# Adamtaranto/mimeo

Measured on AMD Instinct MI355X. Metric: Gbp-aligned/sec (mimeo self, 1 Gbp genome, --minIdt 80 --minLen 100 --minCov 3), higher is better.
Workload: dtype int32

## Files before the change

mimeo_amd/csrc/k6_gapped.hip:

```cpp
#include <algorithm>
#include <cstdio>
#include <cstdlib>
#include <cstring>
#include <vector>

#include "device_util.h"

namespace mimeo {

constexpr int32_t NEG = -(1 << 30);
constexpr int32_t NEGH = -(1 << 29);

struct Cell {
    int32_t s;
    uint32_t nm, nx;
};
struct HalfResult {
    int32_t score;
    uint32_t i, j, nm, nx, overflow;
    uint32_t maxcols, rows;
    uint32_t base_lo, base_hi;
};
struct DpJob {
    uint32_t group, at, aq;
// ... 522 lines not shown
        const int32_t cs = max(hs, is);
        const uint32_t cc = ins ? acc.c : hc;
        const bool take = hs > acc.s;
        acc.c = take ? hc : acc.c;
        acc.s = max(acc.s, hs) - E;
        bool alive = cs >= thr;
        if (EDGE) alive = alive && ((exmask >> s) & 1u);
        S.C[s] = alive ? cs : NEG; S.Cc[s] = cc;
        S.D[s] = alive ? S.D[s] : NEG;
        rowmax = max(rowmax, S.C[s]);
    }
    return rowmax;
}

__device__ HalfResult wave_half_extend_lean(const StrandView &T, const StrandView &Q, uint32_t at, uint32_t aq, int dir,
                                            int32_t O, int32_t E, int32_t Y) {
    const uint32_t lane = threadIdx.x & 63u;
    const uint32_t lenA = dir > 0 ? T.len - at : at, lenB = dir > 0 ? Q.len - aq : aq;
    HalfResult best{0, 0, 0, 0, 0, 0, 0, 0};
    {
        const uint32_t n = min(lenA, lenB);
        const int32_t st = dir > 0 ? (int32_t)at : (int32_t)(at - n), sq = dir > 0 ? (int32_t)aq : (int32_t)(aq - n);
        bool ok = true;
        uint64_t ncg = 0;
        for (uint32_t k0 = 0; k0 < n; k0 += 64u * 32u) {
            uint32_t k = k0 + lane * 32u;
            if (k < n) {
                const Win32 tw = win32(T, st + (int32_t)k), qw = win32(Q, sq + (int32_t)k);
                uint32_t bad = (tw.lo ^ qw.lo) | (tw.hi ^ qw.hi) | tw.nm | qw.nm;
                uint32_t rem = n - k, mask = rem < 32 ? (1u << rem) - 1u : 0xFFFFFFFFu;
                if (bad & mask) ok = false;
                ncg += __popc((tw.lo ^ tw.hi) & mask);
            }
            if (__ballot(!ok)) break;
        }
        if (!__ballot(!ok)) {
            for (int o = 32; o > 0; o >>= 1) ncg += __shfl_xor(ncg, o);
            uint64_t sc = 100ull * ncg + 91ull * ((uint64_t)n - ncg);
            best.score = (int32_t)(uint32_t)sc; best.maxcols = (uint32_t)(sc >> 32); best.i = n; best.j = n; best.nm = n; best.nx = 0;
            return best;
        }
    }
    uint32_t tab[4];
#pragma unroll
    for (uint32_t a = 0; a < 4; a++) {
        uint32_t w = 0;
#pragma unroll
        for (uint32_t b = 0; b < 4; b++) {
            const uint32_t alo = a & 1u, ahi = a >> 1, dl = alo ^ (b & 1u), dh = ahi ^ (b >> 1);
            w |= (uint32_t)(sub_score(dl, dh, alo ^ ahi, 0u) + 128) << (8u * b);
        }
        tab[a] = w;
    }
    LeanState S;
    uint32_t wb = 0, jb = lane * L_WS;
    {
        uint32_t qlo, qhi, qn;
        load_qbits<L_WS>(Q, aq, dir, jb, lenB, qlo, qhi, qn);
        lean_selectors(S, qlo, qhi, qn);
    }
    bool over = false;
#pragma unroll
    for (int s = 0; s < L_WS; s++) {
        const uint32_t j = jb + s;
        const int32_t v = j ? -O - (int32_t)j * E : 0;
        const bool alive = j <= lenB && (j == 0 || v >= -Y);
        S.C[s] = alive ? v : NEG; S.Cc[s] = 0;
        S.D[s] = NEG; S.Dc[s] = 0;
        if (alive && j >= (uint32_t)(L_WINDOW - L_WS)) over = true;
    }
    if (__ballot(over)) { best.overflow = 1; return best; }
    const int32_t lane_base = (int32_t)(lane * L_WS) * E;
    const int32_t kneg128 = __builtin_amdgcn_readfirstlane(-128);
    uint32_t exmask = (1u << L_WS) - 1u;
    bool edge = wb + (uint32_t)L_WINDOW - 1u > lenB;
    if (edge) {
        exmask = 0;
#pragma unroll
        for (int s = 0; s < L_WS; s++) exmask |= (jb + s <= lenB ? 1u : 0u) << s;
    }
    RowBases rbase{0, 0, 0}, rnext = load_row_bases(T, at, dir, 1u);
    for (uint32_t i = 1; i <= lenA; i++) {
        if (i >= 0xFFFFu) { best.overflow = 1; break; }
        const int32_t thr = best.score - Y;
        const uint32_t rbit = (i - 1u) & 31u;
        if (rbit == 0) { rbase = rnext; rnext = load_row_bases(T, at, dir, i + 32u); }
        const uint32_t rlo = (uint32_t)__builtin_amdgcn_readfirstlane((int)rbase.lo), rhi = (uint32_t)__builtin_amdgcn_readfirstlane((int)rbase.hi),
                       rnm = (uint32_t)__builtin_amdgcn_readfirstlane((int)rbase.nm);
        const uint32_t a = ((rlo >> rbit) & 1u) | (((rhi >> rbit) & 1u) << 1);
        uint32_t srow = a & 2u ? (a & 1u ? tab[3] : tab[2]) : (a & 1u ? tab[1] : tab[0]);
        if ((rnm >> rbit) & 1u) srow = 0x1C1C1C1Cu;
        const int32_t rowmax = edge ? lean_row<true>(S, srow, O, E, thr, exmask, lane_base, kneg128)
                                    : lean_row<false>(S, srow, O, E, thr, exmask, lane_base, kneg128);
        const uint64_t ball = __ballot(rowmax > NEGH);
        if (!ball) break;
        const uint32_t rf = (uint32_t)__builtin_ctzll(ball), rl = 63u - (uint32_t)__builtin_clzll(ball);
        if (rl == 63u) { best.overflow = 1; break; }
        best.maxcols = max(best.maxcols, (rl + 1u) * L_WS);
        best.rows = i;
        const int32_t wmax = wave_max_i32(rowmax);
        if (wmax > best.score) {
            const uint32_t L = (uint32_t)__builtin_ctzll(__ballot(rowmax == wmax));
            uint32_t slot = 0, cnt = 0;
#pragma unroll
            for (int s = L_WS - 1; s >= 0; s--) {
                const int32_t v = __builtin_amdgcn_readlane(S.C[s], (int)L);
                if (v == wmax) { slot = (uint32_t)s; cnt = (uint32_t)__builtin_amdgcn_readlane((int)S.Cc[s], (int)L); }
            }
            best.score = wmax; best.i = i; best.j = wb + L * L_WS + slot; best.nm = cnt & 0xFFFFu; best.nx = (cnt >> 16) - (cnt & 0xFFFFu);
        }
        if (rf) {
            wb += rf * L_WS;
            jb = wb + lane * L_WS;
            const int src = (int)((lane + rf) & 63u);
            const bool fresh = lane + rf >= 64u;
#pragma unroll
            for (int s = 0; s < L_WS; s++) {
                const int32_t cs = __shfl(S.C[s], src), ds = __shfl(S.D[s], src);
                S.Cc[s] = __shfl(S.Cc[s], src); S.Dc[s] = __shfl(S.Dc[s], src);
                S.sel[s] = __shfl(S.sel[s], src);
                S.C[s] = fresh ? NEG : cs;
                S.D[s] = fresh ? NEG : ds;
            }
            if (fresh) {
                uint32_t qlo, qhi, qn;
                load_qbits<L_WS>(Q, aq, dir, jb, lenB, qlo, qhi, qn);
                lean_selectors(S, qlo, qhi, qn);
            }
            edge = wb + (uint32_t)L_WINDOW - 1u > lenB;
            if (edge) {
                exmask = 0;
#pragma unroll
                for (int s = 0; s < L_WS; s++) exmask |= (jb + s <= lenB ? 1u : 0u) << s;
            }
        }
    }
    return best;
}

__global__ __launch_bounds__(64) void k6_dp1(const Group *__restrict__ groups, const DpJob *__restrict__ jobs,
                                             HalfResult *__restrict__ res, int32_t O, int32_t E, int32_t Y) {
    const DpJob job = jobs[blockIdx.x];
    const Group &G = groups[job.group];
    HalfResult r = wave_half_extend_lean(G.T, G.Q, job.at, job.aq, job.dir, O, E, Y);
    if (threadIdx.x == 0) res[job.slot] = r;
}

__global__ __launch_bounds__(C4_THREADS) void k6_dp4(const Group *__restrict__ groups, const DpJob *__restrict__ jobs,
                                                     HalfResult *__restrict__ res, int32_t O, int32_t E, int32_t Y) {
    __shared__ C4Shared sh;
    const DpJob job = jobs[blockIdx.x];
    const Group &G = groups[job.group];
    HalfResult r = block_half_extend(sh, G.T, G.Q, job.at, job.aq, job.dir, O, E, Y);
    if (threadIdx.x == 0) res[job.slot] = r;
}

constexpr uint32_t ANCHOR_W = 31, ANCHOR_CHUNK = 4096;
constexpr int ANCHOR_THREADS = 1024;

__device__ void wave_anchor_chunk(const StrandView &T, const StrandView &Q, const mimeo_hsp &h, uint32_t chunk,
                                  unsigned long long *packed) {
    const uint32_t lane = threadIdx.x & 63u, nw = h.length - ANCHOR_W + 1;
    const int32_t d = (int32_t)h.tstart - (int32_t)h.qstart;
    const uint32_t w0 = chunk * ANCHOR_CHUNK + lane * (ANCHOR_CHUNK / 64u), w1 = min(nw, w0 + ANCHOR_CHUNK / 64u);
    int32_t bs = INT32_MIN;
    uint32_t bw = 0xFFFFFFFFu;
    if (w0 < w1) {
        int32_t sum = 0;
        bool m;
        for (uint32_t k = 0; k < ANCHOR_W; k++) {
            int32_t pt = (int32_t)(h.tstart + w0 + k);
            sum += pair_score(T, Q, pt, pt - d, &m);
        }
        bs = sum; bw = w0;
        for (uint32_t w = w0 + 1; w < w1; w++) {
            int32_t add = (int32_t)(h.tstart + w + ANCHOR_W - 1), sub = (int32_t)(h.tstart + w - 1);
            sum += pair_score(T, Q, add, add - d, &m) - pair_score(T, Q, sub, sub - d, &m);
            if (sum > bs) { bs = sum; bw = w; }
        }
    }
    for (int o = 32; o > 0; o >>= 1) {
        int32_t ob = __shfl_xor(bs, o);
        uint32_t ow = __shfl_xor(bw, o);
        if (ob > bs || (ob == bs && ow < bw)) { bs = ob; bw = ow; }
    }
    if (lane == 0 && bw != 0xFFFFFFFFu)
        atomicMax(packed, ((unsigned long long)(uint32_t)(bs + 8192) << 32) | (unsigned long long)(0xFFFFFFFFu - bw));
}

constexpr uint32_t ANCHOR_SPLIT = 16;
__global__ __launch_bounds__(ANCHOR_THREADS) void k6_anchor_points(const Group *__restrict__ groups,
                                                                   const mimeo_hsp *__restrict__ hs,
                                                                   const uint32_t *__restrict__ order,
                                                                   unsigned long long *__restrict__ packed) {
    const Group &G = groups[blockIdx.x];
    const uint64_t b0 = G.hsp_begin;
    const uint32_t nw = gridDim.y * (ANCHOR_THREADS / 64), me = blockIdx.y * (ANCHOR_THREADS / 64) + (threadIdx.x >> 6);
    uint32_t item = 0;
    for (uint32_t r = 0; r < G.nchain; r++) {
        const mimeo_hsp h = hs[b0 + order[b0 + r]];
        if (h.length <= ANCHOR_W) continue;
        const uint32_t nch = (h.length - ANCHOR_W + 1 + ANCHOR_CHUNK - 1) / ANCHOR_CHUNK;
        const uint32_t first = (me + nw - item % nw) % nw;
        for (uint32_t c = first; c < nch; c += nw) wave_anchor_chunk(G.T, G.Q, h, c, &packed[b0 + r]);
        item += nch;
    }
}
__global__ __launch_bounds__(256) void k6_anchor_final(const Group *__restrict__ groups, const mimeo_hsp *__restrict__ hs,
                                                       const uint32_t *__restrict__ order,
                                                       const unsigned long long *__restrict__ packed,
                                                       uint2 *__restrict__ anchors) {
    const Group &G = groups[blockIdx.x];
    const uint64_t b0 = G.hsp_begin;
    for (uint32_t r = threadIdx.x; r < G.nchain; r += blockDim.x) {
        const mimeo_hsp h = hs[b0 + order[b0 + r]];
        uint32_t off = h.length / 2;
        if (h.length > ANCHOR_W) off = (0xFFFFFFFFu - (uint32_t)packed[b0 + r]) + ANCHOR_W / 2;
        anchors[b0 + r] = make_uint2(h.tstart + off, h.qstart + off);
    }
}

__device__ __forceinline__ bool in_boxes(const mimeo_alignment *aln, uint32_t n, uint2 a) {
    bool inside = false;
    for (uint32_t e = threadIdx.x & 63u; e < n; e += 64u) {
        const mimeo_alignment &o = aln[e];
        if (a.x >= o.tstart && a.x < o.tend && a.y >= o.qstart && a.y < o.qend) inside = true;
    }
    return __ballot(inside) != 0;
}

struct PathBlock {
    uint32_t t, q, len;
};
constexpr uint32_t PATH_UNTRACED = 0xFFFFFFFFu;
struct PathView {
    const uint2 *pidx;
    const PathBlock *blk;
    uint32_t *accrank;
};
__device__ __forceinline__ bool on_half_path(const PathBlock *blk, uint32_t n, uint2 a) {
    uint32_t lo = 0, hi = n;
    while (lo < hi) {
        const uint32_t mid = (lo + hi) >> 1;
        if (blk[mid].t <= a.x) lo = mid + 1; else hi = mid;
    }
    if (!lo) return false;
    const PathBlock b = blk[lo - 1];
    return a.x - b.t < b.len && a.y >= b.q && a.y - b.q == a.x - b.t;
}
__device__ __forceinline__ bool on_path(const PathView &P, const uint2 *anchors, uint64_t b0, uint32_t rank, uint2 a) {
    const uint2 an = anchors[b0 + rank];
    const uint2 ix = P.pidx[2u * (b0 + rank) + (a.x >= an.x ? 1u : 0u)];
    if (ix.x == PATH_UNTRACED) return false;
    return on_half_path(P.blk + ix.x, ix.y, a);
}
template <bool PATH>
__device__ __forceinline__ bool skip_test(const mimeo_alignment *aln, uint32_t n, uint2 a, const PathView &P,
                                          const uint2 *anchors, uint64_t b0) {
    if (!PATH) return in_boxes(aln + b0, n, a);
    bool on = false;
    for (uint32_t e = threadIdx.x & 63u; e < n; e += 64u) {
        const mimeo_alignment &o = aln[b0 + e];
        if (a.x >= o.tstart && a.x < o.tend && a.y >= o.qstart && a.y < o.qend && on_path(P, anchors, b0, P.accrank[b0 + e], a))
            on = true;
    }
    return __ballot(on) != 0;
}

enum : uint8_t { A_NEW = 0, A_DONE = 1, A_SKIPPED = 2, A_ACCEPTED = 3 };
constexpr uint32_t PICK_SCAN = 512;
constexpr uint32_t NEAR_DIAG = 256, NEAR_POS = 8192, MAX_DEFER = 2;

__device__ __forceinline__ bool anchors_near(uint2 a, uint2 b) {
    int32_t da = (int32_t)a.x - (int32_t)a.y, db = (int32_t)b.x - (int32_t)b.y;
    uint32_t dd = (uint32_t)abs(da - db), dp = a.x > b.x ? a.x - b.x : b.x - a.x;
    return dd <= NEAR_DIAG && dp <= NEAR_POS;
}

template <bool PATH>
__global__ __launch_bounds__(64) void k6_pick(Group *__restrict__ groups, const uint2 *__restrict__ anchors,
                                              const mimeo_alignment *__restrict__ aln, uint32_t bmax,
                                              uint8_t *__restrict__ astate, uint8_t *__restrict__ adefer,
                                              DpJob *__restrict__ jobs, unsigned int *__restrict__ njobs, PathView P) {
    __shared__ uint32_t sb[MAX_BATCH];
    Group &G = groups[blockIdx.x];
    const uint64_t b0 = G.hsp_begin;
    const uint32_t first = G.next, lane = threadIdx.x;
    uint32_t nb = 0;
    for (uint32_t r = first; r < G.nchain && nb < bmax && r - first < PICK_SCAN; r++) {
        if (astate[b0 + r] != A_NEW) continue;
        const uint2 a = anchors[b0 + r];
        if (skip_test<PATH>(aln, G.nacc, a, P, anchors, b0)) {
            if (lane == 0) astate[b0 + r] = A_SKIPPED;
            continue;
        }
        bool susp = false;
        for (uint32_t r2 = first + lane; r2 < r; r2 += 64)
            if (astate[b0 + r2] == A_DONE && anchors_near(a, anchors[b0 + r2])) susp = true;
        if (lane < nb && anchors_near(a, anchors[b0 + sb[lane]])) susp = true;
        if (__ballot(susp) && adefer[b0 + r] < MAX_DEFER) {
            if (lane == 0) adefer[b0 + r]++;
            continue;
        }
        if (lane == 0) sb[nb] = r;
        nb++;
        __syncthreads();
// ... 481 lines not shown
            m.tid = G.tid; m.qid = G.qid; m.qstrand = G.minus; m.reserved = 0;
            m.tstart = h.tstart; m.tend = h.tstart + h.length; m.qstart = h.qstart; m.qend = h.qstart + h.length;
            m.score = h.score; m.id_n = nmatch; m.id_d = h.length;
            aln[b0 + r] = m;
        }
    }
    if (threadIdx.x == 0) G.nacc = G.nchain;
}

__global__ void k6_finish(Group *__restrict__ groups, uint32_t ngroups, mimeo_alignment *__restrict__ aln,
                          int32_t thresh) {
    uint32_t g = blockIdx.x * blockDim.x + threadIdx.x;
    if (g >= ngroups) return;
    Group &G = groups[g];
    const uint64_t b0 = G.hsp_begin;
    uint32_t k = 0;
    for (uint32_t e = 0; e < G.nacc; e++) {
        mimeo_alignment a = aln[b0 + e];
        if (a.score < thresh) continue;
        if (G.minus) { uint32_t s = G.Q.len - a.qend, t2 = G.Q.len - a.qstart; a.qstart = s; a.qend = t2; }
        aln[b0 + k++] = a;
    }
    G.naln = k;
}

__global__ __launch_bounds__(1024) void k6_dense_offsets(Group *__restrict__ groups, uint32_t ngroups) {
    __shared__ uint32_t part[1024];
    __shared__ uint32_t carry;
    if (threadIdx.x == 0) carry = 0;
    __syncthreads();
    for (uint32_t g0 = 0; g0 < ngroups; g0 += 1024) {
        const uint32_t g = g0 + threadIdx.x, n = g < ngroups ? groups[g].naln : 0u;
        part[threadIdx.x] = n;
        __syncthreads();
        for (uint32_t o = 1; o < 1024; o <<= 1) {
            const uint32_t v = threadIdx.x >= o ? part[threadIdx.x - o] : 0u;
            __syncthreads();
            part[threadIdx.x] += v;
            __syncthreads();
        }
        if (g < ngroups) groups[g].job0 = carry + part[threadIdx.x] - n;
        __syncthreads();
        if (threadIdx.x == 1023) carry += part[1023];
        __syncthreads();
    }
}
__global__ __launch_bounds__(64) void k6_dense_copy(const Group *__restrict__ groups, const mimeo_alignment *__restrict__ aln,
                                                    mimeo_alignment *__restrict__ dense) {
    const Group &G = groups[blockIdx.x];
    for (uint32_t k = threadIdx.x; k < G.naln; k += 64) dense[G.job0 + k] = aln[G.hsp_begin + k];
}
void dense_alignments_device(Group *d_groups, uint32_t ngroups, const mimeo_alignment *d_aln, mimeo_alignment *d_dense) {
    hipLaunchKernelGGL(k6_dense_offsets, dim3(1), dim3(1024), 0, stream(), d_groups, ngroups);
    hipLaunchKernelGGL(k6_dense_copy, dim3(ngroups), dim3(64), 0, stream(), (const Group *)d_groups, d_aln, d_dense);
}

static DeviceBuf g_anchors, g_packed, g_jobs, g_res, g_cnt, g_astate, g_ovf_list, g_any;
static DeviceBuf g_pidx, g_accrank, g_arena, g_pool, g_tjobs, g_tres, g_tctr;

static int trace_pool_budget(uint64_t *budget) {
    size_t free_b = 0, total_b = 0;
    HIP_TRY(hipMemGetInfo(&free_b, &total_b));
    *budget = std::min<uint64_t>(((uint64_t)free_b + g_pool.cap) / 4, 16ull << 30);
    if (getenv("MIMEO_K6_TRACE_POOL_MB")) *budget = (uint64_t)atol(getenv("MIMEO_K6_TRACE_POOL_MB")) << 20;
    return 0;
}

static int arena_reserve(uint64_t blocks, uint64_t used) {
    const size_t bytes = (size_t)blocks * sizeof(PathBlock);
    if (bytes <= g_arena.cap) return 0;
    DeviceBuf nb;
    int rc = nb.reserve(std::max(bytes, 2 * g_arena.cap));
    if (rc) return rc;
    if (used) HIP_TRY(hipMemcpyAsync(nb.p, g_arena.p, (size_t)used * sizeof(PathBlock), hipMemcpyDeviceToDevice, stream()));
    HIP_TRY(hipStreamSynchronize(stream()));
    g_arena.release();
    g_arena = nb;
    return 0;
}

static int trace_round(Group *d_groups, uint32_t h0, const mimeo_params *p, uint64_t budget, uint64_t *arena_used, float *ms,
                       uint32_t *slices, uint64_t *largest) {
    hipStream_t st = stream();
    int rc;
    if ((rc = g_tres.reserve((size_t)h0 * sizeof(HalfResult)))) return rc;
    hipLaunchKernelGGL(k6_trace_gather, dim3((h0 + 255) / 256), dim3(256), 0, st, (const DpJob *)g_jobs.p, h0, (const HalfResult *)g_res.p,
                       (HalfResult *)g_tres.p);
    std::vector<HalfResult> hr(h0);
    HIP_TRY(hipMemcpyAsync(hr.data(), g_tres.p, (size_t)h0 * sizeof(HalfResult), hipMemcpyDeviceToHost, st));
    HIP_TRY(hipStreamSynchronize(st));
    const int32_t O = p->gap_open, E = p->gap_extend, Y = p->ydrop;
    const uint32_t ext = (uint32_t)((Y + 200) / E) + 2u, hi0 = Y >= O + E ? (uint32_t)((Y - O) / E) : 0u;
    std::vector<TraceJob> tj(h0);
    std::vector<uint32_t> cut{0};
    uint64_t fill = 0, need_max = 0, blocks = 0;
    for (uint32_t k = 0; k < h0; k++) {
        const HalfResult &r = hr[k];
        TraceJob J{0, 0, 0, TR_NONE, 0};
        if (!r.overflow && r.i) {
            if (r.rows == 0) { J.mode = TR_DIAG; blocks += 1; }
            else {
                J.W = std::max(r.maxcols, hi0 + 1u) + ext + 2u;
                J.R = 1u;
                while (J.R < J.W + 2u) J.R <<= 1;
                J.cap = std::min(r.i, r.j) + 1u;
                const uint64_t need = trace_layout(r.i, J.W, J.R, J.cap).total;
                *largest = std::max(*largest, need);
                if (need > budget) J.mode = TR_UNTRACED;
                else {
                    J.mode = TR_DP;
                    blocks += J.cap;
                    if (fill + need > budget) { cut.push_back(k); fill = 0; }
                    J.off = fill;
                    fill += need;
                    need_max = std::max(need_max, fill);
                }
            }
        }
        tj[k] = J;
    }
    cut.push_back(h0);
    if ((rc = g_tjobs.reserve((size_t)h0 * sizeof(TraceJob)))) return rc;
    HIP_TRY(hipMemcpyAsync(g_tjobs.p, tj.data(), (size_t)h0 * sizeof(TraceJob), hipMemcpyHostToDevice, st));
    if (need_max && (rc = g_pool.reserve(need_max))) return rc;
    if ((rc = arena_reserve(*arena_used + blocks + 1, *arena_used))) return rc;
    static hipEvent_t e0 = nullptr, e1 = nullptr;
    if (!e0) { HIP_TRY(hipEventCreate(&e0)); HIP_TRY(hipEventCreate(&e1)); }
    HIP_TRY(hipEventRecord(e0, st));
    for (size_t c = 0; c + 1 < cut.size(); c++)
        if (cut[c + 1] > cut[c] && ++*slices)
            hipLaunchKernelGGL(k6_trace, dim3(cut[c + 1] - cut[c]), dim3(TR_THREADS), 0, st, (const Group *)d_groups,
                               (const DpJob *)g_jobs.p, (const TraceJob *)g_tjobs.p, cut[c], (const HalfResult *)g_res.p,
                               (uint8_t *)g_pool.p, (PathBlock *)g_arena.p, (unsigned long long)(g_arena.cap / sizeof(PathBlock)),
                               (uint2 *)g_pidx.p, (unsigned int *)g_tctr.p, O, E, Y);
    HIP_TRY(hipEventRecord(e1, st));
    unsigned int c3[3] = {0, 0, 0};
    HIP_TRY(hipMemcpyAsync(c3, g_tctr.p, 12, hipMemcpyDeviceToHost, st));
    HIP_TRY(hipStreamSynchronize(st));
    float t = 0;
    HIP_TRY(hipEventElapsedTime(&t, e0, e1));
    *ms += t;
    if (c3[1]) {
        char msg[200];
        snprintf(msg, sizeof msg, "internal: K6 traceback of half slot %u %s", c3[2],
                 c3[1] == TRERR_DP ? "disagrees with its DP result (score or end cell)"
                 : c3[1] == TRERR_WALK ? "disagrees with its DP result (matches / mismatches along the path)" : "outgrew the block arena");
        set_error(msg);
        return MIMEO_ERR_ARG;
    }
    *arena_used = c3[0];
    return 0;
}

int gapped_device(Group *d_groups, uint32_t ngroups, const mimeo_hsp *d_sorted, const uint32_t *d_order,
                  uint64_t nhsps, const mimeo_params *p, mimeo_alignment *d_aln) {
    if (!ngroups || !nhsps) return 0;
    hipStream_t st = stream();
    int rc;
    if (!p->gapped) {
        hipLaunchKernelGGL(k6_ungapped, dim3(ngroups), dim3(256), 0, st, d_groups, d_sorted, d_order, d_aln);
    } else {
        uint32_t bmax = 8192u / ngroups;
        if (getenv("MIMEO_K6_BMAX")) bmax = (uint32_t)atoi(getenv("MIMEO_K6_BMAX"));
        const char *kmode = getenv("MIMEO_K6_KERNEL");
        const bool k6_stats = getenv("MIMEO_K6_STATS") != nullptr;
        const int32_t cap = getenv("MIMEO_K6_SCORE_CAP") ? std::max(100000, atoi(getenv("MIMEO_K6_SCORE_CAP"))) : 2000000000;
        bmax = bmax < 1 ? 1 : (bmax > MAX_BATCH ? MAX_BATCH : bmax);
        if ((rc = g_anchors.reserve(nhsps * sizeof(uint2)))) return rc;
        if ((rc = g_packed.reserve(nhsps * 8))) return rc;
        HIP_TRY(hipMemsetAsync(g_packed.p, 0, nhsps * 8, st));
        if ((rc = g_jobs.reserve((size_t)ngroups * bmax * 2 * sizeof(DpJob)))) return rc;
        if ((rc = g_res.reserve((size_t)nhsps * 2 * sizeof(HalfResult)))) return rc;
        if ((rc = g_astate.reserve((size_t)nhsps * 2))) return rc;
        HIP_TRY(hipMemsetAsync(g_astate.p, 0, (size_t)nhsps * 2, st));
        if ((rc = g_cnt.reserve(16))) return rc;
        if ((rc = g_ovf_list.reserve((size_t)ngroups * bmax * 2 * sizeof(unsigned int)))) return rc;
        const uint32_t asplit = ngroups > 4096 ? 1u : ANCHOR_SPLIT;
        hipLaunchKernelGGL(k6_anchor_points, dim3(ngroups, asplit), dim3(ANCHOR_THREADS), 0, st, (const Group *)d_groups,
                           d_sorted, d_order, (unsigned long long *)g_packed.p);
        hipLaunchKernelGGL(k6_anchor_final, dim3(ngroups), dim3(256), 0, st, (const Group *)d_groups, d_sorted, d_order,
                           (const unsigned long long *)g_packed.p, (uint2 *)g_anchors.p);
        const bool path = p->anchor_rule == MIMEO_ANCHOR_PATH;
        uint64_t pool_budget = 0, arena_used = 0;
        float ms_trace = 0;
        uint32_t trace_slices = 0, rounds = 0;
        uint64_t largest = 0;
        PathView pv{nullptr, nullptr, nullptr};
        if (path) {
            if ((rc = g_pidx.reserve((size_t)nhsps * 2 * sizeof(uint2)))) return rc;
            if ((rc = g_accrank.reserve((size_t)nhsps * 4))) return rc;
            if ((rc = g_tctr.reserve(16))) return rc;
            if ((rc = arena_reserve(1024, 0))) return rc;
            HIP_TRY(hipMemsetAsync(g_tctr.p, 0, 16, st));
            if ((rc = trace_pool_budget(&pool_budget))) return rc;
            pv = PathView{(const uint2 *)g_pidx.p, nullptr, (uint32_t *)g_accrank.p};
        }
        for (;;) {
            HIP_TRY(hipMemsetAsync(g_cnt.p, 0, 16, st));
            unsigned int *njobs = (unsigned int *)g_cnt.p, *remaining = njobs + 1, *novf = njobs + 2;
            pv.blk = (const PathBlock *)g_arena.p;
            if (path)
                hipLaunchKernelGGL(k6_pick<true>, dim3(ngroups), dim3(64), 0, st, d_groups, (const uint2 *)g_anchors.p,
                                   (const mimeo_alignment *)d_aln, bmax, (uint8_t *)g_astate.p, (uint8_t *)g_astate.p + nhsps,
                                   (DpJob *)g_jobs.p, njobs, pv);
            else
                hipLaunchKernelGGL(k6_pick<false>, dim3(ngroups), dim3(64), 0, st, d_groups, (const uint2 *)g_anchors.p,
                                   (const mimeo_alignment *)d_aln, bmax, (uint8_t *)g_astate.p, (uint8_t *)g_astate.p + nhsps,
                                   (DpJob *)g_jobs.p, njobs, pv);
            unsigned int h[2] = {0, 0};
            HIP_TRY(hipMemcpyAsync(h, g_cnt.p, 4, hipMemcpyDeviceToHost, st));
            HIP_TRY(hipStreamSynchronize(st));
            if (h[0]) {
                const bool lean_ok = p->gap_extend <= (1 << 16) && p->gap_open <= (1 << 24) && p->ydrop <= (1 << 28);
                if (lean_ok && !kmode) {
                    hipLaunchKernelGGL(k6_dp1, dim3(h[0]), dim3(64), 0, st, (const Group *)d_groups, (const DpJob *)g_jobs.p,
                                       (HalfResult *)g_res.p, p->gap_open, p->gap_extend, p->ydrop);
                } else {
                    const bool use4 = !kmode || !strcmp(kmode, "dp4");
                    if (use4)
                        hipLaunchKernelGGL(k6_dp4, dim3(h[0]), dim3(C4_THREADS), 0, st, (const Group *)d_groups,
                                           (const DpJob *)g_jobs.p, (HalfResult *)g_res.p, p->gap_open, p->gap_extend, p->ydrop);
                    hipLaunchKernelGGL(k6_dp, dim3(h[0]), dim3(64), 0, st, (const Group *)d_groups, (const DpJob *)g_jobs.p,
                                       (HalfResult *)g_res.p, p->gap_open, p->gap_extend, p->ydrop, use4 ? 1 : 0, cap);
                }
                hipLaunchKernelGGL(k6_dp_wide, dim3(h[0]), dim3(64), 0, st, (const Group *)d_groups,
                                   (const DpJob *)g_jobs.p, (HalfResult *)g_res.p, p->gap_open, p->gap_extend, p->ydrop, novf,
                                   (unsigned int *)g_ovf_list.p, cap);
                unsigned int nov = 0;
                HIP_TRY(hipMemcpyAsync(&nov, novf, 4, hipMemcpyDeviceToHost, st));
                HIP_TRY(hipStreamSynchronize(st));
                if (nov) {
                    const unsigned int slots = std::min<unsigned int>(nov, 32u);
                    if ((rc = g_any.reserve((size_t)slots * ANY_SLOT_WORDS * 4))) return rc;
                    for (unsigned int f = 0; f < nov; f += slots)
                        hipLaunchKernelGGL(k6_dp_any, dim3(std::min(slots, nov - f)), dim3(ANY_THREADS), 0, st, (const Group *)d_groups,
                                           (const DpJob *)g_jobs.p, (const unsigned int *)g_ovf_list.p, f, (HalfResult *)g_res.p,
                                           (uint32_t *)g_any.p, p->gap_open, p->gap_extend, p->ydrop, cap);
                }
            }
            if (k6_stats && h[0]) {
                std::vector<DpJob> hj(h[0]);
                std::vector<HalfResult> hall((size_t)nhsps * 2), hr(h[0]);
                HIP_TRY(hipStreamSynchronize(st));
                HIP_TRY(hipMemcpy(hj.data(), g_jobs.p, (size_t)h[0] * sizeof(DpJob), hipMemcpyDeviceToHost));
                HIP_TRY(hipMemcpy(hall.data(), g_res.p, hall.size() * sizeof(HalfResult), hipMemcpyDeviceToHost));
                for (size_t k = 0; k < hr.size(); k++) hr[k] = hall[hj[k].slot];
                unsigned long long hist[9] = {0}, rows = 0, maxr = 0, shortcut = 0;
                for (auto &r : hr) {
                    if (!r.rows) { shortcut++; continue; }
                    hist[std::min<uint32_t>(8, r.maxcols / 128)]++; rows += r.rows; maxr = std::max<unsigned long long>(maxr, r.rows);
                }
                unsigned long long rebased = 0;
                for (auto &r : hr) if (r.base_lo | r.base_hi) rebased++;
                fprintf(stderr, "[k6] jobs %u shortcut %llu (rebased in k6_dp_any: %llu) rows total %llu max %llu band<128..>=1024:", h[0], shortcut, rebased, rows, maxr);
                for (int b = 0; b < 9; b++) fprintf(stderr, " %llu", hist[b]);
                fprintf(stderr, "\n");
                {
                    unsigned long long fine[34] = {0};
                    for (auto &r : hr) if (r.rows) fine[std::min<uint32_t>(33, r.maxcols / 32)]++;
                    fprintf(stderr, "[k6] widest band, buckets of 32 columns from 448:");
                    for (int b = 14; b < 34; b++) fprintf(stderr, " %llu", fine[b]);
                    fprintf(stderr, "\n");
                }
                int shown = 0;
                for (auto &r : hr)
                    if (!r.rows && shown < 8) { fprintf(stderr, "  [k6] zero-row job: score %d i %u j %u nm %u nx %u ovf %u\n", r.score, r.i, r.j, r.nm, r.nx, r.overflow); shown++; }
            }
            if (path && h[0]) {
                rounds++;
                if ((rc = trace_round(d_groups, h[0], p, pool_budget, &arena_used, &ms_trace, &trace_slices, &largest))) return rc;
                pv.blk = (const PathBlock *)g_arena.p;
            }
            if (path)
                hipLaunchKernelGGL(k6_resolve<true>, dim3(ngroups), dim3(64), 0, st, d_groups, (const uint2 *)g_anchors.p,
                                   (const HalfResult *)g_res.p, d_aln, (uint8_t *)g_astate.p, remaining, pv);
            else
                hipLaunchKernelGGL(k6_resolve<false>, dim3(ngroups), dim3(64), 0, st, d_groups, (const uint2 *)g_anchors.p,
                                   (const HalfResult *)g_res.p, d_aln, (uint8_t *)g_astate.p, remaining, pv);
            HIP_TRY(hipMemcpyAsync(h, g_cnt.p, 8, hipMemcpyDeviceToHost, st));
            HIP_TRY(hipStreamSynchronize(st));
            if (!h[1]) break;
        }
        if (path && k6_stats)
            fprintf(stderr, "[k6] path rule: traceback %.3f ms, rounds %u slices %u, %llu path blocks, pool %.1f MB, largest half %.3f MB\n", ms_trace,
                    rounds, trace_slices, (unsigned long long)arena_used, g_pool.cap / 1048576.0, largest / 1048576.0);
    }
    hipLaunchKernelGGL(k6_finish, dim3((ngroups + 63) / 64), dim3(64), 0, st, d_groups, ngroups, d_aln, p->hspthresh);
    HIP_TRY(hipGetLastError());
    return 0;
}

}
```

Before: 0.04243.

## Add four-wave banded DP kernel for rounds with few gapped-extension jobs

Adds k6_dp1w, a 256-thread (four-wave) version of the lean half-extension DP. Each wave owns a 320-column block of a sliding 1280-column window, and the waves exchange boundaries and row maxima through shared memory. It is selected when a round has no more jobs than the device's compute-unit count, so the GPU stays busy in tail rounds where the single-wave kernel leaves most CUs idle. The cost is two block barriers per DP row and more overflow fallbacks when the band outgrows the window.

```diff
diff --git a/mimeo_amd/csrc/k6_gapped.hip b/mimeo_amd/csrc/k6_gapped.hip
--- a/mimeo_amd/csrc/k6_gapped.hip
+++ b/mimeo_amd/csrc/k6_gapped.hip
@@ -698,6 +698,244 @@
     const DpJob job = jobs[blockIdx.x];
     const Group &G = groups[job.group];
     HalfResult r = block_half_extend(sh, G.T, G.Q, job.at, job.aq, job.dir, O, E, Y);
+    if (threadIdx.x == 0) res[job.slot] = r;
+}
+
+constexpr int T_WS = 5, T_BLOCK = 64 * T_WS, T_WINDOW = 4 * T_BLOCK, T_THREADS = 256;
+struct ThinState {
+    int32_t C[T_WS], D[T_WS];
+    uint32_t Cc[T_WS], Dc[T_WS], sel[T_WS];
+};
+struct alignas(16) ThinRecord {
+    uint32_t live;
+    int32_t s;
+    uint32_t j, c;
+};
+struct ThinShared {
+    PCell bnd[4];
+    PCell tot[4];
+    ThinRecord rec[4];
+};
+
+__device__ __forceinline__ void thin_selectors(ThinState &S, const StrandView &Q, uint32_t aq, int dir, uint32_t jb, uint32_t lenB) {
+    uint32_t qlo, qhi, qn;
+    load_qbits<T_WS>(Q, aq, dir, jb, lenB, qlo, qhi, qn);
+#pragma unroll
+    for (int s = 0; s < T_WS; s++) {
+        const uint32_t idx = ((qlo >> s) & 1u) | (((qhi >> s) & 1u) << 1);
+        S.sel[s] = 0x0C0C0C00u | (((qn >> s) & 1u) ? 4u : idx);
+    }
+}
+__device__ __forceinline__ uint32_t thin_exmask(uint32_t jb, uint32_t lenB) {
+    uint32_t m = 0;
+#pragma unroll
+    for (int s = 0; s < T_WS; s++) m |= (jb + s <= lenB ? 1u : 0u) << s;
+    return m;
+}
+
+__device__ __forceinline__ PCell thin_row_h(ThinState &S, PCell pc, uint32_t srow, int32_t O, int32_t E, int32_t lane_base,
+                                            int32_t kneg128) {
+    const int32_t OE = O + E;
+#pragma unroll
+    for (int s = T_WS - 1; s >= 0; s--) {
+        const int32_t t1 = S.D[s] - E, t2 = S.C[s] - OE;
+        const bool open = t2 > t1;
+        const int32_t ds = max(t1, t2);
+        const uint32_t dc = open ? S.Cc[s] : S.Dc[s];
+        const PCell left = s ? PCell{S.C[s ? s - 1 : 0], S.Cc[s ? s - 1 : 0]} : pc;
+        const uint32_t scb = __builtin_amdgcn_perm(28u, srow, S.sel[s]);
+        const int32_t gs = left.s + (int32_t)scb + kneg128;
+        const uint32_t gc = left.c + 0x10000u + ((int32_t)scb > 128 ? 1u : 0u);
+        const bool vert = ds > gs;
+        S.D[s] = ds; S.Dc[s] = dc;
+        S.C[s] = max(gs, ds);
+        S.Cc[s] = vert ? dc : gc;
+    }
+    PCell run{NEG, 0};
+#pragma unroll
+    for (int s = 0; s < T_WS; s++) {
+        const bool take = S.C[s] > run.s;
+        run.c = take ? S.Cc[s] : run.c;
+        run.s = max(run.s, S.C[s]) - E;
+    }
+    run.s += lane_base;
+    return lean_incl_maxscan(run);
+}
+template <bool EDGE>
+__device__ __forceinline__ int32_t thin_row_c(ThinState &S, PCell acc, int32_t O, int32_t E, int32_t thr, uint32_t exmask) {
+    int32_t rowmax = NEG;
+#pragma unroll
+    for (int s = 0; s < T_WS; s++) {
+        const int32_t hs = S.C[s];
+        const uint32_t hc = S.Cc[s];
+        const int32_t is = acc.s - O;
+        const bool ins = is > hs;
+        const int32_t cs = max(hs, is);
+        const uint32_t cc = ins ? acc.c : hc;
+        const bool take = hs > acc.s;
+        acc.c = take ? hc : acc.c;
+        acc.s = max(acc.s, hs) - E;
+        bool alive = cs >= thr;
+        if (EDGE) alive = alive && ((exmask >> s) & 1u);
+        S.C[s] = alive ? cs : NEG; S.Cc[s] = cc;
+        S.D[s] = alive ? S.D[s] : NEG;
+        rowmax = max(rowmax, S.C[s]);
+    }
+    return rowmax;
+}
+
+__device__ HalfResult thin_half_extend(ThinShared &sh, const StrandView &T, const StrandView &Q, uint32_t at, uint32_t aq, int dir,
+                                       int32_t O, int32_t E, int32_t Y) {
+    const uint32_t lane = threadIdx.x & 63u, wave = (uint32_t)__builtin_amdgcn_readfirstlane((int)(threadIdx.x >> 6));
+    const uint32_t lenA = dir > 0 ? T.len - at : at, lenB = dir > 0 ? Q.len - aq : aq;
+    HalfResult best{0, 0, 0, 0, 0, 0, 0, 0};
+    {
+        const uint32_t n = min(lenA, lenB);
+        const int32_t st = dir > 0 ? (int32_t)at : (int32_t)(at - n), sq = dir > 0 ? (int32_t)aq : (int32_t)(aq - n);
+        bool ok = true;
+        uint64_t ncg = 0;
+        for (uint32_t k0 = 0; k0 < n; k0 += 64u * 32u) {
+            uint32_t k = k0 + lane * 32u;
+            if (k < n) {
+                const Win32 tw = win32(T, st + (int32_t)k), qw = win32(Q, sq + (int32_t)k);
+                uint32_t bad = (tw.lo ^ qw.lo) | (tw.hi ^ qw.hi) | tw.nm | qw.nm;
+                uint32_t rem = n - k, mask = rem < 32 ? (1u << rem) - 1u : 0xFFFFFFFFu;
+                if (bad & mask) ok = false;
+                ncg += __popc((tw.lo ^ tw.hi) & mask);
+            }
+            if (__ballot(!ok)) break;
+        }
+        if (!__ballot(!ok)) {
+            for (int o = 32; o > 0; o >>= 1) ncg += __shfl_xor(ncg, o);
+            uint64_t sc = 100ull * ncg + 91ull * ((uint64_t)n - ncg);
+            best.score = (int32_t)(uint32_t)sc; best.maxcols = (uint32_t)(sc >> 32); best.i = n; best.j = n; best.nm = n; best.nx = 0;
+            return best;
+        }
+    }
+    uint32_t tab[4];
+#pragma unroll
+    for (uint32_t a = 0; a < 4; a++) {
+        uint32_t w = 0;
+#pragma unroll
+        for (uint32_t b = 0; b < 4; b++) {
+            const uint32_t alo = a & 1u, ahi = a >> 1, dl = alo ^ (b & 1u), dh = ahi ^ (b >> 1);
+            w |= (uint32_t)(sub_score(dl, dh, alo ^ ahi, 0u) + 128) << (8u * b);
+        }
+        tab[a] = w;
+    }
+    ThinState S;
+    uint32_t wb = 0, wbase = 0;
+    uint32_t rw = wave;
+    uint32_t jb = rw * T_BLOCK + lane * T_WS;
+    thin_selectors(S, Q, aq, dir, jb, lenB);
+    bool over = false;
+#pragma unroll
+    for (int s = 0; s < T_WS; s++) {
+        const uint32_t j = jb + s;
+        const int32_t v = j ? -O - (int32_t)j * E : 0;
+        const bool alive = j <= lenB && (j == 0 || v >= -Y);
+        S.C[s] = alive ? v : NEG; S.Cc[s] = 0;
+        S.D[s] = NEG; S.Dc[s] = 0;
+        if (alive && j >= (uint32_t)(T_WINDOW - T_WS)) over = true;
+    }
+    if (lane == 63) sh.bnd[wave] = PCell{S.C[T_WS - 1], 0};
+    if (__syncthreads_or(over)) { best.overflow = 1; return best; }
+    int32_t lane_base = (int32_t)((rw * 64u + lane) * T_WS) * E;
+    const int32_t kneg128 = __builtin_amdgcn_readfirstlane(-128);
+    bool edge = wb + (rw + 1u) * T_BLOCK - 1u > lenB;
+    uint32_t exmask = thin_exmask(jb, lenB);
+    RowBases rbase{0, 0, 0}, rnext = load_row_bases(T, at, dir, 1u);
+    for (uint32_t i = 1; i <= lenA; i++) {
+        if (i >= 0xFFFFu) { best.overflow = 1; break; }
+        const int32_t thr = best.score - Y;
+        const uint32_t rbit = (i - 1u) & 31u;
+        if (rbit == 0) { rbase = rnext; rnext = load_row_bases(T, at, dir, i + 32u); }
+        const uint32_t rlo = (uint32_t)__builtin_amdgcn_readfirstlane((int)rbase.lo), rhi = (uint32_t)__builtin_amdgcn_readfirstlane((int)rbase.hi),
+                       rnm = (uint32_t)__builtin_amdgcn_readfirstlane((int)rbase.nm);
+        const uint32_t a = ((rlo >> rbit) & 1u) | (((rhi >> rbit) & 1u) << 1);
+        uint32_t srow = a & 2u ? (a & 1u ? tab[3] : tab[2]) : (a & 1u ? tab[1] : tab[0]);
+        if ((rnm >> rbit) & 1u) srow = 0x1C1C1C1Cu;
+        PCell pc = dpp_pcell<0x138, 0xf>(PCell{S.C[T_WS - 1], S.Cc[T_WS - 1]});
+        if (lane == 0 && rw) pc = sh.bnd[(wave + 3u) & 3u];
+        const PCell inc = thin_row_h(S, pc, srow, O, E, lane_base, kneg128);
+        if (lane == 63) sh.tot[rw] = inc;
+        __syncthreads();
+        PCell acc{NEG, 0};
+#pragma unroll
+        for (uint32_t r = 0; r < 3; r++) {
+            const PCell t = sh.tot[r];
+            if (r < rw) acc = pcmax_left(acc, t);
+        }
+        acc = pcmax_left(acc, dpp_pcell<0x138, 0xf>(inc));
+        acc.s += T_WS * E - lane_base;
+        const int32_t rowmax = edge ? thin_row_c<true>(S, acc, O, E, thr, exmask) : thin_row_c<false>(S, acc, O, E, thr, exmask);
+        if (lane == 63) sh.bnd[wave] = PCell{S.C[T_WS - 1], S.Cc[T_WS - 1]};
+        const uint64_t ball = __ballot(rowmax > NEGH);
+        ThinRecord mine{64u, NEG, 0u, 0u};
+        if (ball) mine.live = (uint32_t)__builtin_ctzll(ball) | ((63u - (uint32_t)__builtin_clzll(ball)) << 8);
+        const int32_t wmax = wave_max_i32(rowmax);
+        if (wmax > best.score) {
+            const uint32_t L = (uint32_t)__builtin_ctzll(__ballot(rowmax == wmax));
+            uint32_t slot = 0, cnt = 0;
+#pragma unroll
+            for (int s = T_WS - 1; s >= 0; s--) {
+                const int32_t v = __builtin_amdgcn_readlane(S.C[s], (int)L);
+                if (v == wmax) { slot = (uint32_t)s; cnt = (uint32_t)__builtin_amdgcn_readlane((int)S.Cc[s], (int)L); }
+            }
+            mine.s = wmax; mine.j = wb + rw * T_BLOCK + L * T_WS + slot; mine.c = cnt;
+        }
+        if (lane == 0) sh.rec[rw] = mine;
+        __syncthreads();
+        uint32_t gfirst = 0xFFFFFFFFu, glast = 0;
+        ThinRecord tb{0u, NEG, 0u, 0u};
+#pragma unroll
+        for (uint32_t r = 0; r < 4; r++) {
+            const ThinRecord o = sh.rec[r];
+            const uint32_t live = (uint32_t)__builtin_amdgcn_readfirstlane((int)o.live);
+            const int32_t os = __builtin_amdgcn_readfirstlane(o.s);
+            if ((live & 0xFFu) < 64u) {
+                if (gfirst == 0xFFFFFFFFu) gfirst = r * 64u + (live & 0xFFu);
+                glast = r * 64u + (live >> 8);
+            }
+            if (os > tb.s) {
+                tb.s = os; tb.j = (uint32_t)__builtin_amdgcn_readfirstlane((int)o.j); tb.c = (uint32_t)__builtin_amdgcn_readfirstlane((int)o.c);
+            }
+        }
+        if (gfirst == 0xFFFFFFFFu) break;
+        if (glast == 255u) { best.overflow = 1; break; }
+        best.maxcols = max(best.maxcols, (glast - gfirst + 1u) * T_WS);
+        best.rows = i;
+        if (tb.s > best.score) {
+            best.score = tb.s; best.i = i; best.j = tb.j; best.nm = tb.c & 0xFFFFu; best.nx = (tb.c >> 16) - (tb.c & 0xFFFFu);
+        }
+        const uint32_t k = gfirst >> 6;
+        if (k) {
+            const bool fresh = rw < k;
+            wb += k * T_BLOCK;
+            wbase = (wbase + k) & 3u;
+            rw = (wave - wbase) & 3u;
+            jb = wb + rw * T_BLOCK + lane * T_WS;
+            lane_base = (int32_t)((rw * 64u + lane) * T_WS) * E;
+            if (fresh) {
+#pragma unroll
+                for (int s = 0; s < T_WS; s++) { S.C[s] = NEG; S.D[s] = NEG; }
+                thin_selectors(S, Q, aq, dir, jb, lenB);
+                if (lane == 63) sh.bnd[wave] = PCell{NEG, 0};
+            }
+            edge = wb + (rw + 1u) * T_BLOCK - 1u > lenB;
+            exmask = thin_exmask(jb, lenB);
+            __syncthreads();
+        }
+    }
+    return best;
+}
+
+__global__ __launch_bounds__(T_THREADS) void k6_dp1w(const Group *__restrict__ groups, const DpJob *__restrict__ jobs,
+                                                     HalfResult *__restrict__ res, int32_t O, int32_t E, int32_t Y) {
+    __shared__ ThinShared sh;
+    const DpJob job = jobs[blockIdx.x];
+    const Group &G = groups[job.group];
+    HalfResult r = thin_half_extend(sh, G.T, G.Q, job.at, job.aq, job.dir, O, E, Y);
     if (threadIdx.x == 0) res[job.slot] = r;
 }
 
@@ -1485,6 +1723,17 @@
     return 0;
 }
 
+static unsigned int thin_round_jobs() {
+    static unsigned int t = 0;
+    if (!t) {
+        int dev = 0;
+        hipDeviceProp_t prop;
+        t = (hipGetDevice(&dev) == hipSuccess && hipGetDeviceProperties(&prop, dev) == hipSuccess && prop.multiProcessorCount > 0)
+                ? (unsigned int)prop.multiProcessorCount : 256u;
+    }
+    return t;
+}
+
 int gapped_device(Group *d_groups, uint32_t ngroups, const mimeo_hsp *d_sorted, const uint32_t *d_order,
                   uint64_t nhsps, const mimeo_params *p, mimeo_alignment *d_aln) {
     if (!ngroups || !nhsps) return 0;
@@ -1541,15 +1790,25 @@
                                    (const mimeo_alignment *)d_aln, bmax, (uint8_t *)g_astate.p, (uint8_t *)g_astate.p + nhsps,
                                    (DpJob *)g_jobs.p, njobs, pv);
             unsigned int h[2] = {0, 0};
+            const char *kname = "";
             HIP_TRY(hipMemcpyAsync(h, g_cnt.p, 4, hipMemcpyDeviceToHost, st));
             HIP_TRY(hipStreamSynchronize(st));
             if (h[0]) {
                 const bool lean_ok = p->gap_extend <= (1 << 16) && p->gap_open <= (1 << 24) && p->ydrop <= (1 << 28);
-                if (lean_ok && !kmode) {
-                    hipLaunchKernelGGL(k6_dp1, dim3(h[0]), dim3(64), 0, st, (const Group *)d_groups, (const DpJob *)g_jobs.p,
-                                       (HalfResult *)g_res.p, p->gap_open, p->gap_extend, p->ydrop);
+                const bool force_w = kmode && !strcmp(kmode, "dp1w"), force_1 = kmode && !strcmp(kmode, "dp1");
+                if (lean_ok && (!kmode || force_w || force_1)) {
+                    if (force_w || (!force_1 && h[0] <= thin_round_jobs())) {
+                        kname = "dp1w";
+                        hipLaunchKernelGGL(k6_dp1w, dim3(h[0]), dim3(T_THREADS), 0, st, (const Group *)d_groups, (const DpJob *)g_jobs.p,
+                                           (HalfResult *)g_res.p, p->gap_open, p->gap_extend, p->ydrop);
+                    } else {
+                        kname = "dp1";
+                        hipLaunchKernelGGL(k6_dp1, dim3(h[0]), dim3(64), 0, st, (const Group *)d_groups, (const DpJob *)g_jobs.p,
+                                           (HalfResult *)g_res.p, p->gap_open, p->gap_extend, p->ydrop);
+                    }
                 } else {
                     const bool use4 = !kmode || !strcmp(kmode, "dp4");
+                    kname = use4 ? "dp4" : "dp";
                     if (use4)
                         hipLaunchKernelGGL(k6_dp4, dim3(h[0]), dim3(C4_THREADS), 0, st, (const Group *)d_groups,
                                            (const DpJob *)g_jobs.p, (HalfResult *)g_res.p, p->gap_open, p->gap_extend, p->ydrop);
@@ -1585,7 +1844,7 @@
                 }
                 unsigned long long rebased = 0;
                 for (auto &r : hr) if (r.base_lo | r.base_hi) rebased++;
-                fprintf(stderr, "[k6] jobs %u shortcut %llu (rebased in k6_dp_any: %llu) rows total %llu max %llu band<128..>=1024:", h[0], shortcut, rebased, rows, maxr);
+                fprintf(stderr, "[k6] jobs %u kernel %s shortcut %llu (rebased in k6_dp_any: %llu) rows total %llu max %llu band<128..>=1024:", h[0], kname, shortcut, rebased, rows, maxr);
                 for (int b = 0; b < 9; b++) fprintf(stderr, " %llu", hist[b]);
                 fprintf(stderr, "\n");
                 {
```

Result: no change. 0.04239 (median of 2 runs) (-0.1%).
